# bfs18/nsynth_wavenet

Hardware: AMD Instinct MI355X
Metric: 16 kHz audio samples/sec, parallel-WaveNet (IAF student) generation (higher is better)
Workload: dtype split-fp16: activations stored as fp16 hi+lo pairs (32 bits per value, 22-bit significand, fp16 exponent range), contractions as 3 fp16 MFMAs per product with fp32 accumulate; conditioning term and outputs fp32; 1 GPU; BASELINE.json configs[1]: parallel_wavenet.json IAF student generation, synthetic 80-dim mel, 16 kHz, 1 utterance(s) of 384 frames = 76800 samples per GPU per step; batch_per_gpu=1, frames=384, samples_per_utterance=76800, weights=random-init (TF initialisers), seed 1234; noise drawn on device (Philox), precision=f16x3, parallelism=utterance-sharded x1 (no data-path collective)

## Files before the change

nsynth_wavenet_amd/csrc/wn_deconv.hip:

```cpp
#include <algorithm>

#include "wn_internal.h"
#include "wn_codec.h"
#include "wn_pack_h.h"
#include "wn_mfma_h.h"


namespace {

constexpr int DC_NT = 4;
constexpr int DC_QT = 16 * DC_NT;
constexpr int DC_XOFF = 8;
constexpr int DC_QW = 256;
constexpr int DH_KC = 4;

__host__ __device__ inline int dc_row_stride(int L) {
    return DC_XOFF + ((L + 5 + DC_QW - 1) / DC_QW) * DC_QW + 8;
}

__global__ void mel_to_cm_kernel(const float* __restrict__ mel, float* __restrict__ out,
                                 int F, int C, int xs) {
    const int b = blockIdx.z, c = blockIdx.y;
    const int col = blockIdx.x * blockDim.x + threadIdx.x;
    if (col >= xs) return;
    const int f = col - DC_XOFF;
    float v = 0.f;
    if (f >= 0 && f < F) v = mel[((size_t)b * F + f) * C + c];
    out[((size_t)b * C + c) * xs + col] = v;
}

__device__ inline float apply_act(float v, int act) {
    if (act == WN_ACT_LEAKY_RELU) return fmaxf(v, 0.4f * v);
    if (act == WN_ACT_RELU) return fmaxf(v, 0.f);
    return tanhf(v);
}

__global__ __launch_bounds__(256) void deconv_mfma_kernel(
    const float* __restrict__ x, int cin, int xs, const float* __restrict__ wp,
    float* __restrict__ yp, int cout, int Qp, int S, int taps, int zc_count) {
    const int lane = threadIdx.x & 63, wave = threadIdx.x >> 6;
    const int n = lane & 15, kq = lane >> 4;
    const int r = blockIdx.y;
    const int b = blockIdx.z / zc_count, zc = blockIdx.z % zc_count;
    const int cg = zc * 4 + wave;
    if (cg * 64 >= cout) return;
    const int q0 = blockIdx.x * DC_QT;
    const int nmb = cout / 16;
    const int cblk = cin / 16;
    const int nks4 = taps * cblk;

    f4 acc[4][DC_NT];
#pragma unroll
    for (int mb = 0; mb < 4; ++mb)
#pragma unroll
        for (int e = 0; e < DC_NT; ++e) acc[mb][e] = (f4){0.f, 0.f, 0.f, 0.f};

    const f4* wpr = reinterpret_cast<const f4*>(wp) + ((size_t)r * nks4 * nmb + cg * 4) * 64 + lane;
    const float* xb = x + (size_t)b * cin * xs + DC_XOFF + q0 + DC_NT * n;

    auto load = [&](int it, f4 (&a)[4], f4 (&bv)[4]) {
        const int j = it / cblk, c4 = it - j * cblk;
#pragma unroll
        for (int mb = 0; mb < 4; ++mb) a[mb] = wpr[((size_t)it * nmb + mb) * 64];
#pragma unroll
        for (int jj = 0; jj < 4; ++jj)
            bv[jj] = *reinterpret_cast<const f4u*>(xb + (size_t)(16 * c4 + 4 * jj + kq) * xs - j);
    };
    f4 a1[4], b1[4];
    load(0, a1, b1);
    for (int it = 0; it < nks4; ++it) {
        f4 a[4], bv[4];
#pragma unroll
        for (int i = 0; i < 4; ++i) { a[i] = a1[i]; bv[i] = b1[i]; }
        if (it + 1 < nks4) load(it + 1, a1, b1);
#pragma unroll
        for (int jj = 0; jj < 4; ++jj)
#pragma unroll
            for (int mb = 0; mb < 4; ++mb)
#pragma unroll
                for (int e = 0; e < DC_NT; ++e)
                    acc[mb][e] = __builtin_amdgcn_mfma_f32_16x16x4f32(a[mb][jj], bv[jj][e], acc[mb][e], 0, 0, 0);
    }
#pragma unroll
    for (int mb = 0; mb < 4; ++mb)
#pragma unroll
        for (int rr = 0; rr < 4; ++rr) {
            const int co = 64 * cg + 16 * mb + 4 * kq + rr;
            float* row = yp + (((size_t)b * S + r) * cout + co) * Qp + q0 + DC_NT * n;
            *reinterpret_cast<f4*>(row) = (f4){acc[mb][0][rr], acc[mb][1][rr], acc[mb][2][rr], acc[mb][3][rr]};
        }
}

constexpr int DI_MAXS = 32;
__global__ __launch_bounds__(256) void deconv_interleave_kernel(
    const float* __restrict__ yp, const float* __restrict__ bias, float* __restrict__ y,
    int cout, int Qp, int64_t ys, int yoff, int L, int S, int pL, int act) {
    __shared__ float tile[DI_MAXS][DC_QT + 1];
    const int co = blockIdx.y, b = blockIdx.z;
    const int q0 = blockIdx.x * DC_QT;
    for (int i = threadIdx.x; i < S * DC_QT; i += 256) {
        const int r = i / DC_QT, q = i - r * DC_QT;
        tile[r][q] = yp[(((size_t)b * S + r) * cout + co) * Qp + q0 + q];
    }
    __syncthreads();
    const float bco = bias[co];
    const int64_t SL = (int64_t)S * L;
    float* yr = y + ((size_t)b * cout + co) * ys + yoff;
    const int64_t n0 = (int64_t)S * q0 - pL;
    for (int i = threadIdx.x; i < S * DC_QT; i += 256) {
        const int q = i / S, r = i - q * S;
        const int64_t nn = n0 + i;
        if (nn >= 0 && nn < SL) yr[nn] = apply_act(tile[r][q] + bco, act);
    }
}

__global__ void mel_to_split_kernel(const float* __restrict__ mel, unsigned* __restrict__ out,
                                    int F, int C, int xs, unsigned* __restrict__ status) {
    const int b = blockIdx.z, cp = blockIdx.y;
    const int col = blockIdx.x * blockDim.x + threadIdx.x;
    if (col >= xs) return;
    const int f = col - DC_XOFF;
    unsigned hw = 0, lw = 0;
    if (f >= 0 && f < F) {
        const float* m = mel + ((size_t)b * F + f) * C + 2 * cp;
        float amax = 0.f;
        wn_split_pair_t(m[0], m[1], hw, lw, amax);
        wn_range_flag(amax, status);
    }
    out[((size_t)b * C + cp) * xs + col] = hw;
    out[((size_t)b * C + C / 2 + cp) * xs + col] = lw;
}

template <bool G4IN>
__global__ __launch_bounds__(256, 2) void deconv_mfma_h_kernel(
    const unsigned* __restrict__ x, int cin, int xs, const unsigned* __restrict__ wp,
    float* __restrict__ yp, int cout, int Qp, int S, int taps, float inv_scale) {
    __shared__ __attribute__((aligned(16))) unsigned lds[2][DH_KC * 4 * 512];
    const int lane = threadIdx.x & 63, wave = threadIdx.x >> 6;
    const int n = lane & 15, kg = lane >> 4;
    const int r = blockIdx.y;
    const int ncg = cout / 64;
    const int b = blockIdx.z / ncg, cg = blockIdx.z % ncg;
    const int q0 = blockIdx.x * DC_QW + wave * DC_QT;
    const int nmb = cout / 16;
    const int nb16 = cin / 16;
    const int nks = taps * nb16 / 2;
    const int nchunk = (nks + DH_KC - 1) / DH_KC;

    f4 acc[4][DC_NT];
#pragma unroll
    for (int mb = 0; mb < 4; ++mb)
#pragma unroll
        for (int e = 0; e < DC_NT; ++e) acc[mb][e] = (f4){0.f, 0.f, 0.f, 0.f};

    const wn_u4* wsrc = reinterpret_cast<const wn_u4*>(wp);
    auto stage = [&](int chunk, int buf) {
#pragma unroll
        for (int kl = 0; kl < DH_KC; ++kl) {
            const int ks = chunk * DH_KC + kl;
            if (ks < nks) {
                const wn_u4* src = wsrc + (((size_t)r * nks + ks) * nmb + cg * 4) * 128;
                wn_u4* dst = reinterpret_cast<wn_u4*>(lds[buf]) + kl * 512;
                dst[threadIdx.x] = src[threadIdx.x];
                dst[threadIdx.x + 256] = src[threadIdx.x + 256];
            }
        }
    };
    const unsigned* xb = x + (size_t)b * cin * xs;
    const size_t lo_plane = (size_t)(cin / 2) * xs;
    auto loadB = [&](int ks, wn_u4 (&vh)[DC_NT], wn_u4 (&vl)[DC_NT]) {
        if (G4IN) {
            const int nb32 = cin / 32;
            const int j = ks / nb32, c = ks - j * nb32;
            const unsigned* p = xb + ((size_t)(4 * c + kg) * xs + DC_XOFF + q0 + DC_NT * n - j) * 4;
#pragma unroll
            for (int e = 0; e < DC_NT; ++e) {
                vh[e] = *reinterpret_cast<const wn_u4*>(p + 4 * e);
                vl[e] = *reinterpret_cast<const wn_u4*>(p + lo_plane + 4 * e);
            }
        } else {
            wn_u4 bh[4], bl[4];
#pragma unroll
            for (int i = 0; i < 4; ++i) {
                const int g = 2 * ks + (i >> 1);
                const int j = g / nb16, blk = g - j * nb16;
                const unsigned* p = xb + (size_t)(8 * blk + 2 * kg + (i & 1)) * xs + DC_XOFF + q0 + DC_NT * n - j;
                bh[i] = *reinterpret_cast<const wn_u4 __attribute__((aligned(4)))*>(p);
                bl[i] = *reinterpret_cast<const wn_u4 __attribute__((aligned(4)))*>(p + lo_plane);
            }
#pragma unroll
            for (int e = 0; e < DC_NT; ++e) {
                vh[e] = (wn_u4){bh[0][e], bh[1][e], bh[2][e], bh[3][e]};
                vl[e] = (wn_u4){bl[0][e], bl[1][e], bl[2][e], bl[3][e]};
            }
        }
    };

    stage(0, 0);
    wn_u4 b1h[DC_NT], b1l[DC_NT];
    loadB(0, b1h, b1l);
    __syncthreads();
    for (int chunk = 0; chunk < nchunk; ++chunk) {
        const int buf = chunk & 1;
        if (chunk + 1 < nchunk) stage(chunk + 1, buf ^ 1);
        const wn_u4* Al = reinterpret_cast<const wn_u4*>(lds[buf]) + lane;
#pragma unroll
        for (int kl = 0; kl < DH_KC; ++kl) {
            const int ks = chunk * DH_KC + kl;
            if (ks >= nks) break;
            wn_u4 vh[DC_NT], vl[DC_NT];
#pragma unroll
            for (int e = 0; e < DC_NT; ++e) { vh[e] = b1h[e]; vl[e] = b1l[e]; }
            if (ks + 1 < nks) loadB(ks + 1, b1h, b1l);
#pragma unroll
            for (int mb = 0; mb < 4; ++mb) {
                const wn_u4 ah = Al[(kl * 4 + mb) * 128], al = Al[(kl * 4 + mb) * 128 + 64];
#pragma unroll
                for (int e = 0; e < DC_NT; ++e) {
                    f4 c = acc[mb][e];
                    c = __builtin_amdgcn_mfma_f32_16x16x32_f16(__builtin_bit_cast(wn_h8, ah), __builtin_bit_cast(wn_h8, vh[e]), c, 0, 0, 0);
                    c = __builtin_amdgcn_mfma_f32_16x16x32_f16(__builtin_bit_cast(wn_h8, ah), __builtin_bit_cast(wn_h8, vl[e]), c, 0, 0, 0);
                    c = __builtin_amdgcn_mfma_f32_16x16x32_f16(__builtin_bit_cast(wn_h8, al), __builtin_bit_cast(wn_h8, vh[e]), c, 0, 0, 0);
                    acc[mb][e] = c;
                }
            }
        }
        __syncthreads();
    }
#pragma unroll
    for (int mb = 0; mb < 4; ++mb)
#pragma unroll
        for (int rr = 0; rr < 4; ++rr) {
            const int co = 64 * cg + 16 * mb + 4 * kg + rr;
            float* row = yp + (((size_t)b * S + r) * cout + co) * Qp + q0 + DC_NT * n;
            *reinterpret_cast<f4*>(row) = (f4){acc[mb][0][rr] * inv_scale, acc[mb][1][rr] * inv_scale,
                                               acc[mb][2][rr] * inv_scale, acc[mb][3][rr] * inv_scale};
        }
}

__device__ inline unsigned dpp_shr1(unsigned old, unsigned src) {
    return (unsigned)__builtin_amdgcn_update_dpp((int)old, (int)src, 0x111, 0xf, 0xf, false);
}

template <int TAPS>
__global__ __launch_bounds__(256, 2) void deconv_mfma_hs_kernel(
    const unsigned* __restrict__ x, int cin, int xs, const unsigned* __restrict__ wp,
    float* __restrict__ yp, int cout, int Qp, int S, float inv_scale) {
    constexpr int taps = TAPS, NH = TAPS > 1 ? TAPS - 1 : 1;
    __shared__ __attribute__((aligned(16))) unsigned lds[2][DH_KC * 4 * 512];
    const int lane = threadIdx.x & 63, wave = threadIdx.x >> 6;
    const int n = lane & 15, kg = lane >> 4;
    const int r = blockIdx.y;
    const int ncg = cout / 64;
    const int b = blockIdx.z / ncg, cg = blockIdx.z % ncg;
    const int q0 = blockIdx.x * DC_QW + wave * DC_QT;
    const int nmb = cout / 16;
    const int nb32 = cin / 32;
    const int nks = taps * nb32;
    constexpr int ntg = (taps + DH_KC - 1) / DH_KC;
    const int nchunk = nb32 * ntg;

    f4 acc[4][DC_NT];
#pragma unroll
    for (int mb = 0; mb < 4; ++mb)
#pragma unroll
        for (int e = 0; e < DC_NT; ++e) acc[mb][e] = (f4){0.f, 0.f, 0.f, 0.f};

    const wn_u4* wsrc = reinterpret_cast<const wn_u4*>(wp);
    wn_u4 wt[DH_KC][2];
    auto stage_load = [&](int chunk) {
        const int c = chunk / ntg, tg = chunk - c * ntg;
#pragma unroll
        for (int kl = 0; kl < DH_KC; ++kl) {
            const int j = tg * DH_KC + kl;
            if (j < taps) {
                const wn_u4* src = wsrc + (((size_t)r * nks + j * nb32 + c) * nmb + cg * 4) * 128;
                wt[kl][0] = src[threadIdx.x];
                wt[kl][1] = src[threadIdx.x + 256];
            }
        }
    };
    auto stage_store = [&](int chunk, int buf) {
        const int c = chunk / ntg, tg = chunk - c * ntg;
#pragma unroll
        for (int kl = 0; kl < DH_KC; ++kl) {
            if (tg * DH_KC + kl < taps) {
                wn_u4* dst = reinterpret_cast<wn_u4*>(lds[buf]) + kl * 512;
                dst[threadIdx.x] = wt[kl][0];
                dst[threadIdx.x + 256] = wt[kl][1];
            }
        }
    };
    const unsigned* xb = x + (size_t)b * cin * xs;
    const size_t lo_plane = (size_t)(cin / 2) * xs;
    auto loadB = [&](int c, wn_u4 (&vh)[DC_NT], wn_u4 (&vl)[DC_NT], wn_u4 (&hh)[NH], wn_u4 (&hl)[NH]) {
        const unsigned* row = xb + ((size_t)(4 * c + kg) * xs + DC_XOFF + q0) * 4;
        const unsigned* p = row + DC_NT * n * 4;
#pragma unroll
        for (int e = 0; e < DC_NT; ++e) {
            vh[e] = *reinterpret_cast<const wn_u4*>(p + 4 * e);
            vl[e] = *reinterpret_cast<const wn_u4*>(p + lo_plane + 4 * e);
        }
#pragma unroll
        for (int k = 0; k + 1 < taps; ++k) {
            hh[k] = *reinterpret_cast<const wn_u4*>(row - 4 * (k + 1));
            hl[k] = *reinterpret_cast<const wn_u4*>(row + lo_plane - 4 * (k + 1));
        }
    };

    stage_load(0);
    stage_store(0, 0);
    wn_u4 nh[DC_NT], nl[DC_NT], nhh[NH], nhl[NH];
    loadB(0, nh, nl, nhh, nhl);
    __syncthreads();
    wn_u4 vh[DC_NT], vl[DC_NT], hh[NH], hl[NH];
    for (int c = 0; c < nb32; ++c) {
#pragma unroll
        for (int e = 0; e < DC_NT; ++e) { vh[e] = nh[e]; vl[e] = nl[e]; }
#pragma unroll
        for (int k = 0; k < NH; ++k) { hh[k] = nhh[k]; hl[k] = nhl[k]; }
        if (c + 1 < nb32) loadB(c + 1, nh, nl, nhh, nhl);
#pragma unroll
      for (int tg = 0; tg < ntg; ++tg) {
        const int chunk = c * ntg + tg;
        const int buf = chunk & 1;
        if (chunk + 1 < nchunk) stage_load(chunk + 1);
        const wn_u4* Al = reinterpret_cast<const wn_u4*>(lds[buf]) + lane;
#pragma unroll
        for (int kl = 0; kl < DH_KC; ++kl) {
            const int j = tg * DH_KC + kl;
            if (j < taps) {
            if (j > 0) {
                const wn_u4 th = vh[DC_NT - 1], tl = vl[DC_NT - 1];
#pragma unroll
                for (int e = DC_NT - 1; e > 0; --e) { vh[e] = vh[e - 1]; vl[e] = vl[e - 1]; }
                const wn_u4 oh = hh[j > 0 ? j - 1 : 0], ol = hl[j > 0 ? j - 1 : 0];
#pragma unroll
                for (int i = 0; i < 4; ++i) {
                    vh[0][i] = dpp_shr1(oh[i], th[i]);
                    vl[0][i] = dpp_shr1(ol[i], tl[i]);
                }
            }
#pragma unroll
            for (int mb = 0; mb < 4; ++mb) {
                const wn_u4 ah = Al[(kl * 4 + mb) * 128], al = Al[(kl * 4 + mb) * 128 + 64];
#pragma unroll
                for (int e = 0; e < DC_NT; ++e) {
                    f4 cc = acc[mb][e];
                    cc = __builtin_amdgcn_mfma_f32_16x16x32_f16(__builtin_bit_cast(wn_h8, ah), __builtin_bit_cast(wn_h8, vh[e]), cc, 0, 0, 0);
                    cc = __builtin_amdgcn_mfma_f32_16x16x32_f16(__builtin_bit_cast(wn_h8, ah), __builtin_bit_cast(wn_h8, vl[e]), cc, 0, 0, 0);
                    cc = __builtin_amdgcn_mfma_f32_16x16x32_f16(__builtin_bit_cast(wn_h8, al), __builtin_bit_cast(wn_h8, vh[e]), cc, 0, 0, 0);
                    acc[mb][e] = cc;
                }
            }
            }
        }
        if (chunk + 1 < nchunk) stage_store(chunk + 1, buf ^ 1);
        __syncthreads();
      }
    }
#pragma unroll
    for (int mb = 0; mb < 4; ++mb)
#pragma unroll
        for (int rr = 0; rr < 4; ++rr) {
            const int co = 64 * cg + 16 * mb + 4 * kg + rr;
            float* row = yp + (((size_t)b * S + r) * cout + co) * Qp + q0 + DC_NT * n;
            *reinterpret_cast<f4*>(row) = (f4){acc[mb][0][rr] * inv_scale, acc[mb][1][rr] * inv_scale,
                                               acc[mb][2][rr] * inv_scale, acc[mb][3][rr] * inv_scale};
        }
}

constexpr int PG_TP = 4;
constexpr int PG_NT = 5;
constexpr int PG_WAVES = 8;
constexpr int PG_FRAMES = PG_WAVES * 16 * PG_NT;
constexpr int PG_KS_WORDS = 8 * 2 * 64 * 4;
constexpr int PG_RG_WORDS_PER_BLOCK = PG_TP * PG_KS_WORDS;
constexpr int PG_LDS_BYTES = 2 * PG_RG_WORDS_PER_BLOCK * 4;
constexpr int PG_MAXG = 8;

struct PgArgs {
    const unsigned* x;
    int cin, xs, L;
    const unsigned* wp;
    const float* bias;
    float inv_scale;
    unsigned* y;
    int cout, S, act;
    int64_t ys;
    int yoff;
    unsigned* status;
    int ntiles;
    int ngroups, nrg;
    int g_p0[PG_MAXG], g_nph[PG_MAXG], g_d[PG_MAXG], g_rg0[PG_MAXG];
};

__device__ inline void pg_dma16(const unsigned* gsrc, unsigned lds_byte_addr) {
    unsigned keep;
    asm volatile("s_mov_b32 %0, m0\n\ts_mov_b32 m0, %2\n\ts_nop 0\n\tglobal_load_lds_dwordx4 %1, off\n\ts_mov_b32 m0, %0"
                 : "=&s"(keep) : "v"(gsrc), "s"(__builtin_amdgcn_readfirstlane(lds_byte_addr)) : "memory");
}

__global__ __launch_bounds__(PG_WAVES * 64, 1) void deconv_pg_kernel(const PgArgs A) {
    extern __shared__ __attribute__((aligned(16))) unsigned pg_lds[];
    char* lds = reinterpret_cast<char*>(pg_lds);
    const unsigned lds_base = __builtin_amdgcn_readfirstlane((unsigned)(size_t)(__attribute__((address_space(3))) char*)lds);
    constexpr int NT = PG_NT, TP = PG_TP, NR = NT + TP - 1;
    int rg, tile;
    if ((A.nrg & 7) == 0) {
        const int k = blockIdx.x >> 3;
        rg = (blockIdx.x & 7) + 8 * (k / A.ntiles);
        tile = k % A.ntiles;
    } else {
        rg = blockIdx.x / A.ntiles;
        tile = blockIdx.x % A.ntiles;
    }
    int gi = 0;
    for (int k = 1; k < A.ngroups; ++k) if (rg >= A.g_rg0[k]) gi = k;
    const int p0 = A.g_p0[gi], nph = A.g_nph[gi], dcol = A.g_d[gi], sub = rg - A.g_rg0[gi];
    const int b = blockIdx.y;
    const int lane = threadIdx.x & 63, wave = __builtin_amdgcn_readfirstlane(threadIdx.x >> 6);
    const int n = lane & 15, kg = lane >> 4;
    const int nb32 = A.cin / 32, ngi = A.cin / 8, ngo = A.cout / 8;
    const int f0 = tile * PG_FRAMES + wave * (16 * NT);
    const unsigned* wsrc = A.wp + (size_t)rg * nb32 * PG_RG_WORDS_PER_BLOCK;

    f4 acc[8][NT];
#pragma unroll
    for (int mb = 0; mb < 8; ++mb)
#pragma unroll
        for (int e = 0; e < NT; ++e) acc[mb][e] = (f4){0.f, 0.f, 0.f, 0.f};

    auto stage = [&](int c, int buf) {
        const unsigned* src = wsrc + (size_t)c * PG_RG_WORDS_PER_BLOCK;
#pragma unroll
        for (int i = 0; i < PG_RG_WORDS_PER_BLOCK / 256 / PG_WAVES; ++i) {
            const int piece = wave * (PG_RG_WORDS_PER_BLOCK / 256 / PG_WAVES) + i;
            pg_dma16(src + (size_t)(piece * 64 + lane) * 4, lds_base + buf * (PG_RG_WORDS_PER_BLOCK * 4) + piece * 1024);
        }
    };
    const __amdgpu_buffer_rsrc_t rx = __builtin_amdgcn_make_buffer_rsrc(
        (void*)(A.x + (size_t)b * 2 * ngi * A.xs * 4), 0, 2 * ngi * A.xs * 16, 0x00020000);
    const int lo_plane = ngi * A.xs * 16;
    wn_u4 Rh[NR], Rl[NR];
    auto loadB = [&](int c) {
        const int vo = (4 * c + kg) * A.xs * 16 + (DC_XOFF + f0 + NT * n + dcol - (TP - 1)) * 16;
#pragma unroll
        for (int k = 0; k < NR; ++k) {
            Rh[k] = __builtin_bit_cast(wn_u4, __builtin_amdgcn_raw_buffer_load_b128(rx, vo + k * 16, 0, 0));
            Rl[k] = __builtin_bit_cast(wn_u4, __builtin_amdgcn_raw_buffer_load_b128(rx, vo + k * 16, lo_plane, 0));
        }
    };

    stage(0, 0);
    loadB(0);
    asm volatile("s_waitcnt vmcnt(0)" ::: "memory");
    __syncthreads();
    for (int c = 0; c < nb32; ++c) {
        const int buf = c & 1;
        if (c + 1 < nb32) stage(c + 1, buf ^ 1);
#pragma unroll
        for (int m = 0; m < TP; ++m) {
            const wn_u4* Al = reinterpret_cast<const wn_u4*>(lds + buf * (PG_RG_WORDS_PER_BLOCK * 4)) + m * (PG_KS_WORDS / 4) + lane;
#pragma unroll
            for (int mb = 0; mb < 8; ++mb) {
                const wn_u4 ah = Al[mb * 128], al = Al[mb * 128 + 64];
#pragma unroll
                for (int e = 0; e < NT; ++e) {
                    const wn_u4 bh = Rh[e + TP - 1 - m], bl = Rl[e + TP - 1 - m];
                    f4 cc = acc[mb][e];
                    cc = __builtin_amdgcn_mfma_f32_16x16x32_f16(__builtin_bit_cast(wn_h8, ah), __builtin_bit_cast(wn_h8, bh), cc, 0, 0, 0);
                    cc = __builtin_amdgcn_mfma_f32_16x16x32_f16(__builtin_bit_cast(wn_h8, ah), __builtin_bit_cast(wn_h8, bl), cc, 0, 0, 0);
                    cc = __builtin_amdgcn_mfma_f32_16x16x32_f16(__builtin_bit_cast(wn_h8, al), __builtin_bit_cast(wn_h8, bh), cc, 0, 0, 0);
                    acc[mb][e] = cc;
                }
            }
        }
        if (c + 1 < nb32) loadB(c + 1);
        asm volatile("s_waitcnt vmcnt(0)" ::: "memory");
        __syncthreads();
    }
    const __amdgpu_buffer_rsrc_t ry = __builtin_amdgcn_make_buffer_rsrc(
        (void*)(A.y + (size_t)b * 2 * ngo * A.ys * 4), 0, (int)(2 * ngo * A.ys * 16), 0x00020000);
    const int lo_out = (int)(ngo * A.ys * 16);
    float amax = 0.f;
    const bool half = nph == 2;
    const int cb_first = half ? 4 * sub : 2 * sub;
    float bs[4][4];
#pragma unroll
    for (int k = 0; k < 4; ++k)
#pragma unroll
        for (int rr = 0; rr < 4; ++rr) bs[k][rr] = (half || k < 2) ? A.bias[16 * (cb_first + k) + 4 * kg + rr] : 0.f;
    char* patch = lds + wave * 8192;
    const int fr = f0 + NT * (lane >> 2);
    const int w2r = lane & 3;
    const int phr = half ? (w2r & 1) : w2r, sgr = half ? (w2r >> 1) : 0;
#pragma unroll
    for (int e = 0; e < NT; ++e) {
#pragma unroll
        for (int w2 = 0; w2 < 4; ++w2) {
            wn_u4 hw, lw;
#pragma unroll
            for (int slot = 0; slot < 4; ++slot) {
                const int blk = slot >> 1, r0 = (slot & 1) * 2;
                const float a0 = half ? acc[(4 * (w2 & 1) + 2 * (w2 >> 1) + blk) & 7][e][r0] : acc[(2 * w2 + blk) & 7][e][r0];
                const float a1 = half ? acc[(4 * (w2 & 1) + 2 * (w2 >> 1) + blk) & 7][e][r0 + 1] : acc[(2 * w2 + blk) & 7][e][r0 + 1];
                const float b0 = half ? bs[2 * (w2 >> 1) + blk][r0] : bs[blk][r0];
                const float b1 = half ? bs[2 * (w2 >> 1) + blk][r0 + 1] : bs[blk][r0 + 1];
                const float v0 = apply_act(fmaf(a0, A.inv_scale, b0), A.act);
                const float v1 = apply_act(fmaf(a1, A.inv_scale, b1), A.act);
                unsigned a, c2;
                wn_split_pair_t(v0, v1, a, c2, amax);
                hw[slot] = a;
                lw[slot] = c2;
            }
            *reinterpret_cast<wn_u4*>(patch + ((kg * 16 + n) * 4 + w2) * 16) = hw;
            *reinterpret_cast<wn_u4*>(patch + 4096 + ((kg * 16 + n) * 4 + w2) * 16) = lw;
        }
        const int f = fr + e;
        const int64_t tcol = A.yoff + (int64_t)A.S * f + p0 + phr;
#pragma unroll
        for (int kr = 0; kr < 4; ++kr) {
            const int g = 4 * ((cb_first >> 1) + sgr) + kr;
            const int vo = f < A.L ? (int)(((int64_t)g * A.ys + tcol) * 16) : (int)0x80000000;
            const wn_u4 hw = *reinterpret_cast<const wn_u4*>(patch + (kr * 64 + lane) * 16);
            const wn_u4 lw = *reinterpret_cast<const wn_u4*>(patch + 4096 + (kr * 64 + lane) * 16);
            buf_st4(hw, ry, vo, 0);
            buf_st4(lw, ry, vo, lo_out);
        }
    }
    wn_range_flag(amax, A.status);
}

__global__ void cm_to_tm_kernel(const float* __restrict__ in, float* __restrict__ out,
                                int C, int64_t T, int64_t cs) {
    __shared__ float tile[32][33];
    const int b = blockIdx.z;
    const int64_t t0 = (int64_t)blockIdx.x * 32;
    const int c0 = blockIdx.y * 32;
    const int tx = threadIdx.x & 31, ty = threadIdx.x >> 5;
    for (int i = ty; i < 32; i += 8) {
        const int c = c0 + i;
        const int64_t t = t0 + tx;
        tile[i][tx] = (c < C && t < T) ? in[((size_t)b * C + c) * cs + t] : 0.f;
    }
    __syncthreads();
    for (int i = ty; i < 32; i += 8) {
        const int64_t t = t0 + i;
        const int c = c0 + tx;
        if (t < T && c < C) out[((size_t)b * T + t) * C + c] = tile[tx][i];
    }
}

constexpr int DG_Q = 32;
template <int SC>
__global__ __launch_bounds__(256) void deconv_interleave_g4_kernel(
    const float* __restrict__ yp, const float* __restrict__ bias, unsigned* __restrict__ y,
    int cout, int Qp, int64_t ys, int yoff, int L, int S_rt, int pL, int act, unsigned* __restrict__ status,
    int zero_pads) {
    const int S = SC ? SC : S_rt;
    __shared__ float tile[8][DI_MAXS][DG_Q + 1];
    const int g = blockIdx.y, b = blockIdx.z;
    const int q0 = blockIdx.x * DG_Q;
    if (zero_pads && (blockIdx.x == 0 || blockIdx.x + 1 == gridDim.x)) {
        wn_u4* rh = reinterpret_cast<wn_u4*>(y + ((size_t)b * cout * ys)) + (size_t)g * ys;
        wn_u4* rl = rh + (size_t)(cout / 8) * ys;
        const int64_t lo = blockIdx.x == 0 ? 0 : yoff + (int64_t)S * L, hi = blockIdx.x == 0 ? yoff : ys;
        for (int64_t i = lo + threadIdx.x; i < hi; i += 256) rh[i] = rl[i] = (wn_u4){0u, 0u, 0u, 0u};
    }
    const int prbase = 16 * (g >> 2) + 2 * (g & 3);
    for (int i = threadIdx.x; i < 8 * S * (DG_Q / 4); i += 256) {
        const int c8 = i / (S * (DG_Q / 4)), j = i - c8 * S * (DG_Q / 4);
        const int r = j / (DG_Q / 4), q = 4 * (j - r * (DG_Q / 4));
        const int slot = c8 >> 1;
        const int ch = 2 * (prbase + 8 * (slot >> 1) + (slot & 1)) + (c8 & 1);
        const f4 v = *reinterpret_cast<const f4*>(yp + (((size_t)b * S + r) * cout + ch) * Qp + q0 + q);
#pragma unroll
        for (int k = 0; k < 4; ++k) tile[c8][r][q + k] = v[k];
    }
    __syncthreads();
    float bs[8];
#pragma unroll
    for (int c8 = 0; c8 < 8; ++c8) {
        const int slot = c8 >> 1;
        bs[c8] = bias[2 * (prbase + 8 * (slot >> 1) + (slot & 1)) + (c8 & 1)];
    }
    const int ng = cout / 8;
    const int64_t SL = (int64_t)S * L;
    wn_u4* yh = reinterpret_cast<wn_u4*>(y + ((size_t)b * cout * ys)) + (size_t)g * ys + yoff;
    wn_u4* yl = yh + (size_t)ng * ys;
    const int64_t n0 = (int64_t)S * q0 - pL;
    float amax = 0.f;
    for (int i = threadIdx.x; i < S * DG_Q; i += 256) {
        const int q = i / S, r = i - q * S;
        const int64_t nn = n0 + i;
        if (nn >= 0 && nn < SL) {
            wn_u4 hw, lw;
#pragma unroll
            for (int slot = 0; slot < 4; ++slot) {
                unsigned a, c2;
                wn_split_pair_t(apply_act(tile[2 * slot][r][q] + bs[2 * slot], act),
                                apply_act(tile[2 * slot + 1][r][q] + bs[2 * slot + 1], act), a, c2, amax);
                hw[slot] = a;
                lw[slot] = c2;
            }
            yh[nn] = hw;
            yl[nn] = lw;
        }
    }
    wn_range_flag(amax, status);
}

constexpr int DF_WAVES = 8;
constexpr int DF_CIN = 80;
constexpr int DF_NKS = 4 * (DF_CIN / 16) / 2;
constexpr int DF_WIN = 16 + 3;
constexpr int DF_PF = 3;

__device__ inline float mul_round_add(float a, float s, float b) {
#pragma clang fp contract(off)
    const float m = a * s;
    return m + b;
}

struct FrontArgs {
    const float* mel;
    int B, F;
    const unsigned* wp;
    const float* bias;
    float inv_scale;
    unsigned* y;
    int ys;
    int S, pL, act;
    int ncb, nunits;
    unsigned* status;
};

__global__ __launch_bounds__(DF_WAVES * 64) void deconv_front_kernel(const FrontArgs A) {
    __shared__ __attribute__((aligned(16))) unsigned win[2][DF_WIN][DF_CIN / 2];
    const int u = (blockIdx.x & 7) * (gridDim.x >> 3) + (blockIdx.x >> 3);
    if (u >= A.nunits) return;
    const int cb = u % A.ncb, pb = u / A.ncb;
    const int b = pb % A.B, p = pb / A.B;
    const int r = (p + A.pL) % A.S, d = (p + A.pL) / A.S;
    const int lane = threadIdx.x & 63, wave = __builtin_amdgcn_readfirstlane(threadIdx.x >> 6);
    const int n = lane & 15, kg = lane >> 4;
    const int f0 = 16 * cb;
    constexpr int ng = 32, nmb = 16;

    const float* melb = A.mel + (size_t)b * A.F * DF_CIN;
    constexpr int NP = (DF_WIN * (DF_CIN / 2) + DF_WAVES * 64 - 1) / (DF_WAVES * 64);
    wn_f2 mv[NP];
    bool mok[NP];
#pragma unroll
    for (int k = 0; k < NP; ++k) {
        const int i = threadIdx.x + k * DF_WAVES * 64;
        const int fl = i / (DF_CIN / 2), pr = i - fl * (DF_CIN / 2);
        const int fr = f0 + d - 3 + fl;
        mok[k] = fl < DF_WIN && fr >= 0 && fr < A.F;
        mv[k] = *reinterpret_cast<const wn_f2 __attribute__((aligned(4)))*>(melb + (size_t)min(max(fr, 0), A.F - 1) * DF_CIN + 2 * pr);
    }
    f4 bs[2];
#pragma unroll
    for (int mb = 0; mb < 2; ++mb) bs[mb] = *reinterpret_cast<const f4u*>(A.bias + 32 * wave + 16 * mb + 4 * kg);
    const wn_u4* wsrc = reinterpret_cast<const wn_u4*>(A.wp) + ((size_t)r * DF_NKS * nmb + 2 * wave) * 128 + lane;
    wn_u4 ah[DF_NKS][2], al[DF_NKS][2];
    auto loadA = [&](int ks) {
#pragma unroll
        for (int mb = 0; mb < 2; ++mb) {
            ah[ks][mb] = wsrc[(ks * nmb + mb) * 128];
            al[ks][mb] = wsrc[(ks * nmb + mb) * 128 + 64];
        }
        __builtin_amdgcn_sched_barrier(0);
    };
#pragma unroll
    for (int ks = 0; ks < DF_PF; ++ks) loadA(ks);
    float amax = 0.f;
#pragma unroll
    for (int k = 0; k < NP; ++k) {
        const int i = threadIdx.x + k * DF_WAVES * 64;
        const int fl = i / (DF_CIN / 2), pr = i - fl * (DF_CIN / 2);
        if (fl < DF_WIN) {
            unsigned hw = 0, lw = 0;
            if (mok[k]) wn_split_pair_t(mv[k].x, mv[k].y, hw, lw, amax);
            win[0][fl][pr] = hw;
            win[1][fl][pr] = lw;
        }
    }
    __syncthreads();

    f4 acc[2];
    acc[0] = acc[1] = (f4){0.f, 0.f, 0.f, 0.f};
#pragma unroll
    for (int ks = 0; ks < DF_NKS; ++ks) {
        if (ks + DF_PF < DF_NKS) loadA(ks + DF_PF);
        wn_u4 vh, vl;
#pragma unroll
        for (int i = 0; i < 4; ++i) {
            const int g = 2 * ks + (i >> 1);
            const int j = g / (DF_CIN / 16), blk = g - j * (DF_CIN / 16);
            vh[i] = win[0][n + 3 - j][8 * blk + 2 * kg + (i & 1)];
            vl[i] = win[1][n + 3 - j][8 * blk + 2 * kg + (i & 1)];
        }
#pragma unroll
        for (int mb = 0; mb < 2; ++mb) {
            f4 c = acc[mb];
            c = __builtin_amdgcn_mfma_f32_16x16x32_f16(__builtin_bit_cast(wn_h8, ah[ks][mb]), __builtin_bit_cast(wn_h8, vh), c, 0, 0, 0);
            c = __builtin_amdgcn_mfma_f32_16x16x32_f16(__builtin_bit_cast(wn_h8, ah[ks][mb]), __builtin_bit_cast(wn_h8, vl), c, 0, 0, 0);
            c = __builtin_amdgcn_mfma_f32_16x16x32_f16(__builtin_bit_cast(wn_h8, al[ks][mb]), __builtin_bit_cast(wn_h8, vh), c, 0, 0, 0);
            acc[mb] = c;
        }
    }

    const __amdgpu_buffer_rsrc_t ry = __builtin_amdgcn_make_buffer_rsrc(
        (void*)(A.y + (size_t)b * 2 * ng * A.ys * 4), 0, 2 * ng * A.ys * 16, 0x00020000);
    const int lo_out = ng * A.ys * 16;
    wn_u4 hw, lw;
#pragma unroll
    for (int slot = 0; slot < 4; ++slot) {
        const int mb = slot >> 1, r0 = (slot & 1) * 2;
        const float v0 = apply_act(mul_round_add(acc[mb][r0], A.inv_scale, bs[mb][r0]), A.act);
        const float v1 = apply_act(mul_round_add(acc[mb][r0 + 1], A.inv_scale, bs[mb][r0 + 1]), A.act);
        unsigned a, c2;
        wn_split_pair_t(v0, v1, a, c2, amax);
        hw[slot] = a;
        lw[slot] = c2;
    }
    const int f = f0 + n;
    {
        const int vo = f < A.F ? ((4 * wave + kg) * A.ys + DC_XOFF + A.S * f + p) * 16 : (int)0x80000000;
        buf_st4(hw, ry, vo, 0);
        buf_st4(lw, ry, vo, lo_out);
    }
    wn_range_flag(amax, A.status);
    if (cb + 1 == A.ncb) {
        const int SL = A.S * A.F, nz = A.ys - SL;
        for (int row = p; row < 2 * ng; row += A.S)
            for (int i = threadIdx.x; i < nz; i += DF_WAVES * 64)
                buf_st4((wn_u4){0u, 0u, 0u, 0u}, ry, (row * A.ys + (i < DC_XOFF ? i : SL + i)) * 16, 0);
    }
}

}

int wn_pack_deconv(wn_handle* h, std::vector<float>& blob) {
    const wn_config& c = h->cfg;
    for (auto& sp : h->stacks) {
        int cin = c.n_mel;
        for (int j = 0; j < c.n_deconv; ++j) {
            DeconvLayerPack lp;
            lp.cin = cin;
            lp.cout = c.deconv_width;
            lp.K = c.deconv_filter[j];
            lp.S = c.deconv_stride[j];
            lp.pL = (lp.K - lp.S) / 2;
            lp.taps = lp.K / lp.S;
            if (cin % 16) return wn_fail(h, WN_EINVAL, "deconv: input channels %d not a multiple of 16", cin);
            std::string scope = (sp.prefix.empty() ? std::string() : sp.prefix + "/") +
                                (c.use_resize_conv ? "resize_conv_" : "trans_conv_") + std::to_string(j + 1);
            std::vector<float> W;
            if (c.use_resize_conv) {
                const int fl = lp.K, S = lp.S;
                std::vector<float> Wr = wn_get_kernel(h, scope, "W", false);
                int taps = (fl - 1 + S - 1) / S + 1;
                if ((taps * (cin / 16)) % 2) ++taps;
                lp.taps = taps;
                lp.K = S * taps;
                lp.pL = fl - 1 - (fl - 1) / 2;
                W.assign((size_t)lp.K * lp.cout * cin, 0.f);
                for (int r = 0; r < S; ++r)
                    for (int k = 0; k < fl; ++k) {
                        const int m = r + k - (fl - 1);
                        const int jt = m >= 0 ? 0 : (-m + S - 1) / S;
                        for (int co = 0; co < lp.cout; ++co)
                            for (int ci = 0; ci < cin; ++ci)
                                W[((size_t)(S * jt + r) * lp.cout + co) * cin + ci] +=
                                    Wr[((size_t)k * cin + ci) * lp.cout + co];
                    }
            } else {
                W = wn_get_kernel(h, scope, "kernel", true);
            }
            const std::vector<float>& bias = h->vars.at(scope + (c.use_resize_conv ? "/biases" : "/bias")).data;
            const int nmb = lp.cout / 16, cblk = cin / 16, nks4 = lp.taps * cblk;
            blob.resize(align_up(blob.size(), 64));
// ... 388 lines not shown
```

Measured before the change: 64.91 million samples/s.

## Interleave next-chunk register loads with MFMA taps in deconv main loop

After: 64.97 million samples/s, median of 6. Within noise of the previous version (+0.1%).

```diff
diff --git a/nsynth_wavenet_amd/csrc/wn_deconv.hip b/nsynth_wavenet_amd/csrc/wn_deconv.hip
--- a/nsynth_wavenet_amd/csrc/wn_deconv.hip
+++ b/nsynth_wavenet_amd/csrc/wn_deconv.hip
@@ -395,10 +395,10 @@
     int g_p0[PG_MAXG], g_nph[PG_MAXG], g_d[PG_MAXG], g_rg0[PG_MAXG];
 };
 
-__device__ inline void pg_dma16(const unsigned* gsrc, unsigned lds_byte_addr) {
+__device__ inline void pg_dma16(const unsigned* sbase, unsigned lane_byte_off, unsigned lds_byte_addr) {
     unsigned keep;
-    asm volatile("s_mov_b32 %0, m0\n\ts_mov_b32 m0, %2\n\ts_nop 0\n\tglobal_load_lds_dwordx4 %1, off\n\ts_mov_b32 m0, %0"
-                 : "=&s"(keep) : "v"(gsrc), "s"(__builtin_amdgcn_readfirstlane(lds_byte_addr)) : "memory");
+    asm volatile("s_mov_b32 %0, m0\n\ts_mov_b32 m0, %3\n\ts_nop 0\n\tglobal_load_lds_dwordx4 %1, %2\n\ts_mov_b32 m0, %0"
+                 : "=&s"(keep) : "v"(lane_byte_off), "s"(sbase), "s"(__builtin_amdgcn_readfirstlane(lds_byte_addr)) : "memory");
 }
 
 __global__ __launch_bounds__(PG_WAVES * 64, 1) void deconv_pg_kernel(const PgArgs A) {
@@ -436,49 +436,64 @@
 #pragma unroll
         for (int i = 0; i < PG_RG_WORDS_PER_BLOCK / 256 / PG_WAVES; ++i) {
             const int piece = wave * (PG_RG_WORDS_PER_BLOCK / 256 / PG_WAVES) + i;
-            pg_dma16(src + (size_t)(piece * 64 + lane) * 4, lds_base + buf * (PG_RG_WORDS_PER_BLOCK * 4) + piece * 1024);
+            pg_dma16(src + (size_t)piece * 256, lane * 16, lds_base + buf * (PG_RG_WORDS_PER_BLOCK * 4) + piece * 1024);
         }
     };
     const __amdgpu_buffer_rsrc_t rx = __builtin_amdgcn_make_buffer_rsrc(
         (void*)(A.x + (size_t)b * 2 * ngi * A.xs * 4), 0, 2 * ngi * A.xs * 16, 0x00020000);
     const int lo_plane = ngi * A.xs * 16;
     wn_u4 Rh[NR], Rl[NR];
-    auto loadB = [&](int c) {
-        const int vo = (4 * c + kg) * A.xs * 16 + (DC_XOFF + f0 + NT * n + dcol - (TP - 1)) * 16;
-#pragma unroll
-        for (int k = 0; k < NR; ++k) {
-            Rh[k] = __builtin_bit_cast(wn_u4, __builtin_amdgcn_raw_buffer_load_b128(rx, vo + k * 16, 0, 0));
-            Rl[k] = __builtin_bit_cast(wn_u4, __builtin_amdgcn_raw_buffer_load_b128(rx, vo + k * 16, lo_plane, 0));
-        }
+    constexpr int OOB = 0x40000000;
+    const int vo0 = kg * A.xs * 16 + (DC_XOFF + f0 + NT * n + dcol - (TP - 1)) * 16;
+    auto loadR = [&](int c, int k) {
+        const int vo = vo0 + 4 * c * A.xs * 16 + k * 16 + (c < nb32 ? 0 : OOB);
+        Rh[k] = __builtin_bit_cast(wn_u4, __builtin_amdgcn_raw_buffer_load_b128(rx, vo, 0, 0));
+        Rl[k] = __builtin_bit_cast(wn_u4, __builtin_amdgcn_raw_buffer_load_b128(rx, vo, lo_plane, 0));
+        __builtin_amdgcn_sched_barrier(0);
     };
+    auto mfma_tap = [&](int m, int mb, int e, const wn_u4& ah, const wn_u4& al) {
+        const wn_u4 bh = Rh[e + TP - 1 - m], bl = Rl[e + TP - 1 - m];
+        f4 cc = acc[mb][e];
+        cc = __builtin_amdgcn_mfma_f32_16x16x32_f16(__builtin_bit_cast(wn_h8, ah), __builtin_bit_cast(wn_h8, bh), cc, 0, 0, 0);
+        cc = __builtin_amdgcn_mfma_f32_16x16x32_f16(__builtin_bit_cast(wn_h8, ah), __builtin_bit_cast(wn_h8, bl), cc, 0, 0, 0);
+        cc = __builtin_amdgcn_mfma_f32_16x16x32_f16(__builtin_bit_cast(wn_h8, al), __builtin_bit_cast(wn_h8, bh), cc, 0, 0, 0);
+        acc[mb][e] = cc;
+    };
 
     stage(0, 0);
-    loadB(0);
+#pragma unroll
+    for (int k = 0; k < NR; ++k) loadR(0, k);
     asm volatile("s_waitcnt vmcnt(0)" ::: "memory");
     __syncthreads();
+    auto tap_part = [&](const wn_u4* Al, int m, int e0, int e1, int rot) {
+#pragma unroll
+        for (int mb = 0; mb < 8; ++mb) {
+            const wn_u4 ah = Al[mb * 128], al = Al[mb * 128 + 64];
+#pragma unroll
+            for (int i = 0; i < e1 - e0; ++i) mfma_tap(m, mb, e0 + (i + rot) % (e1 - e0), ah, al);
+        }
+    };
+    constexpr int EH3 = 3;
     for (int c = 0; c < nb32; ++c) {
         const int buf = c & 1;
+        const wn_u4* Ab = reinterpret_cast<const wn_u4*>(lds + buf * (PG_RG_WORDS_PER_BLOCK * 4)) + lane;
+        tap_part(Ab, 0, 0, NT, 2);
+        loadR(c + 1, NR - 1);
         if (c + 1 < nb32) stage(c + 1, buf ^ 1);
-#pragma unroll
-        for (int m = 0; m < TP; ++m) {
-            const wn_u4* Al = reinterpret_cast<const wn_u4*>(lds + buf * (PG_RG_WORDS_PER_BLOCK * 4)) + m * (PG_KS_WORDS / 4) + lane;
-#pragma unroll
-            for (int mb = 0; mb < 8; ++mb) {
-                const wn_u4 ah = Al[mb * 128], al = Al[mb * 128 + 64];
-#pragma unroll
-                for (int e = 0; e < NT; ++e) {
-                    const wn_u4 bh = Rh[e + TP - 1 - m], bl = Rl[e + TP - 1 - m];
-                    f4 cc = acc[mb][e];
-                    cc = __builtin_amdgcn_mfma_f32_16x16x32_f16(__builtin_bit_cast(wn_h8, ah), __builtin_bit_cast(wn_h8, bh), cc, 0, 0, 0);
-                    cc = __builtin_amdgcn_mfma_f32_16x16x32_f16(__builtin_bit_cast(wn_h8, ah), __builtin_bit_cast(wn_h8, bl), cc, 0, 0, 0);
-                    cc = __builtin_amdgcn_mfma_f32_16x16x32_f16(__builtin_bit_cast(wn_h8, al), __builtin_bit_cast(wn_h8, bh), cc, 0, 0, 0);
-                    acc[mb][e] = cc;
-                }
-            }
-        }
-        if (c + 1 < nb32) loadB(c + 1);
-        asm volatile("s_waitcnt vmcnt(0)" ::: "memory");
-        __syncthreads();
+        tap_part(Ab + PG_KS_WORDS / 4, 1, 0, NT, 0);
+        loadR(c + 1, NR - 2);
+        tap_part(Ab + 2 * (PG_KS_WORDS / 4), 2, 0, NT, 0);
+        loadR(c + 1, NR - 3);
+        tap_part(Ab + 3 * (PG_KS_WORDS / 4), 3, 0, EH3, 0);
+        asm volatile("" ::: "memory");
+#pragma unroll
+        for (int k = 0; k < EH3; ++k) loadR(c + 1, k);
+        tap_part(Ab + 3 * (PG_KS_WORDS / 4), 3, EH3, NT, 0);
+#pragma unroll
+        for (int k = EH3; k < NT; ++k) loadR(c + 1, k);
+        asm volatile("s_waitcnt vmcnt(4)" ::: "memory");
+        __builtin_amdgcn_s_barrier();
+        asm volatile("" ::: "memory");
     }
     const __amdgpu_buffer_rsrc_t ry = __builtin_amdgcn_make_buffer_rsrc(
         (void*)(A.y + (size_t)b * 2 * ngo * A.ys * 4), 0, (int)(2 * ngo * A.ys * 16), 0x00020000);
```

## Software-pipeline deconv main loop with per-slot window reloads and scheduled MFMA groups

Applied to the files above, without the earlier changes.

Result: no change. 66.09 million samples/s before, 66.12 million samples/s after (median of 6 runs) (+0.0%).

```diff
diff --git a/nsynth_wavenet_amd/csrc/wn_deconv.hip b/nsynth_wavenet_amd/csrc/wn_deconv.hip
--- a/nsynth_wavenet_amd/csrc/wn_deconv.hip
+++ b/nsynth_wavenet_amd/csrc/wn_deconv.hip
@@ -1,4 +1,6 @@
 #include <algorithm>
+#include <type_traits>
+#include <utility>
 
 #include "wn_internal.h"
 #include "wn_codec.h"
@@ -378,6 +380,46 @@
 constexpr int PG_RG_WORDS_PER_BLOCK = PG_TP * PG_KS_WORDS;
 constexpr int PG_LDS_BYTES = 2 * PG_RG_WORDS_PER_BLOCK * 4;
 constexpr int PG_MAXG = 8;
+constexpr int PG_DMA_PER_WAVE = PG_RG_WORDS_PER_BLOCK / 256 / PG_WAVES;
+constexpr int PG_STEPS = 40;
+constexpr int PG_DMA_STEP = 3;
+constexpr int pg_step_tap(int s) { return s < 24 ? s / 8 : PG_TP - 1; }
+constexpr int pg_step_e0(int s) { return s >= 24 && s < 32 ? 3 : 0; }
+constexpr int pg_step_e1(int s) { return s >= 32 ? 3 : PG_NT; }
+constexpr int pg_slot_reload_step(int k) { return k == 7 ? 7 : k == 6 ? 15 : k == 5 ? 23 : k >= 3 ? 31 : PG_STEPS - 1; }
+constexpr bool pg_step_reads_slot(int s, int k) {
+    return k >= pg_step_e0(s) + PG_TP - 1 - pg_step_tap(s) && k < pg_step_e1(s) + PG_TP - 1 - pg_step_tap(s);
+}
+constexpr bool pg_reloads_are_dead() {
+    for (int k = 0; k < PG_NT + PG_TP - 1; ++k)
+        for (int s = pg_slot_reload_step(k) + 1; s < PG_STEPS; ++s)
+            if (pg_step_reads_slot(s, k)) return false;
+    return true;
+}
+constexpr bool pg_steps_cover_the_tile() {
+    for (int m = 0; m < PG_TP; ++m)
+        for (int e = 0; e < PG_NT; ++e) {
+            int n = 0;
+            for (int s = 0; s < PG_STEPS; s += 8) n += pg_step_tap(s) == m && e >= pg_step_e0(s) && e < pg_step_e1(s);
+            if (n != 1) return false;
+        }
+    return true;
+}
+static_assert(PG_TP == 4 && PG_NT == 5, "the step table above is written for four taps and five column blocks");
+static_assert(pg_reloads_are_dead(),"a window slot is reloaded in front of a step of the same stage that reads it");
+static_assert(pg_steps_cover_the_tile(), "the steps do not cover (tap, column block) exactly once");
+static_assert(PG_STEPS % 2 == 0, "the fragment pairs rotate with the step parity across stages");
+constexpr int pg_slots_reloaded_behind(int s) {
+    int n = 0;
+    for (int k = 0; k < PG_NT + PG_TP - 1; ++k) n += pg_slot_reload_step(k) == s;
+    return n;
+}
+template <int... S, class F>
+__device__ inline void pg_static_for(std::integer_sequence<int, S...>, F&& f) {
+    (f(std::integral_constant<int, S>{}), ...);
+}
+constexpr int PG_B_LOADS = 2 * (PG_NT + PG_TP - 1);
+static_assert(PG_DMA_STEP < pg_slot_reload_step(PG_NT + PG_TP - 2), "a window reload is issued in front of the LDS-DMA requests");
 
 struct PgArgs {
     const unsigned* x;
@@ -432,54 +474,82 @@
         for (int e = 0; e < NT; ++e) acc[mb][e] = (f4){0.f, 0.f, 0.f, 0.f};
 
     auto stage = [&](int c, int buf) {
-        const unsigned* src = wsrc + (size_t)c * PG_RG_WORDS_PER_BLOCK;
-#pragma unroll
-        for (int i = 0; i < PG_RG_WORDS_PER_BLOCK / 256 / PG_WAVES; ++i) {
-            const int piece = wave * (PG_RG_WORDS_PER_BLOCK / 256 / PG_WAVES) + i;
-            pg_dma16(src + (size_t)(piece * 64 + lane) * 4, lds_base + buf * (PG_RG_WORDS_PER_BLOCK * 4) + piece * 1024);
-        }
+        const unsigned* src = wsrc + (size_t)c * PG_RG_WORDS_PER_BLOCK + wave * (PG_DMA_PER_WAVE * 256);
+#pragma unroll
+        for (int i = 0; i < PG_DMA_PER_WAVE; ++i)
+            pg_dma16(src + i * 256 + lane * 4, lds_base + buf * (PG_RG_WORDS_PER_BLOCK * 4) + (wave * PG_DMA_PER_WAVE + i) * 1024);
     };
     const __amdgpu_buffer_rsrc_t rx = __builtin_amdgcn_make_buffer_rsrc(
         (void*)(A.x + (size_t)b * 2 * ngi * A.xs * 4), 0, 2 * ngi * A.xs * 16, 0x00020000);
     const int lo_plane = ngi * A.xs * 16;
     wn_u4 Rh[NR], Rl[NR];
-    auto loadB = [&](int c) {
-        const int vo = (4 * c + kg) * A.xs * 16 + (DC_XOFF + f0 + NT * n + dcol - (TP - 1)) * 16;
-#pragma unroll
-        for (int k = 0; k < NR; ++k) {
-            Rh[k] = __builtin_bit_cast(wn_u4, __builtin_amdgcn_raw_buffer_load_b128(rx, vo + k * 16, 0, 0));
-            Rl[k] = __builtin_bit_cast(wn_u4, __builtin_amdgcn_raw_buffer_load_b128(rx, vo + k * 16, lo_plane, 0));
-        }
+    const int vo0 = kg * A.xs * 16 + (DC_XOFF + f0 + NT * n + dcol - (TP - 1)) * 16, vo_step = 4 * A.xs * 16;
+    int vo = vo0;
+    auto loadB = [&](int k) {
+        Rh[k] = __builtin_bit_cast(wn_u4, __builtin_amdgcn_raw_buffer_load_b128(rx, vo + k * 16, 0, 0));
+        Rl[k] = __builtin_bit_cast(wn_u4, __builtin_amdgcn_raw_buffer_load_b128(rx, vo + k * 16, lo_plane, 0));
     };
+    const wn_u4* Al = reinterpret_cast<const wn_u4*>(lds) + lane;
+    wn_u4 ah[2], al[2];
+    auto loadA = [&](int buf, int s) {
+        const wn_u4* p = Al + buf * (PG_RG_WORDS_PER_BLOCK / 4) + pg_step_tap(s) * (PG_KS_WORDS / 4) + (s & 7) * 128;
+        ah[s & 1] = p[0];
+        al[s & 1] = p[64];
+    };
 
     stage(0, 0);
-    loadB(0);
+#pragma unroll
+    for (int k = NR - 1; k >= 0; --k)
+        if (pg_slot_reload_step(k) != PG_STEPS - 1) loadB(k);
+    __builtin_amdgcn_sched_barrier(0);
+#pragma unroll
+    for (int k = NR - 1; k >= 0; --k)
+        if (pg_slot_reload_step(k) == PG_STEPS - 1) loadB(k);
     asm volatile("s_waitcnt vmcnt(0)" ::: "memory");
     __syncthreads();
-    for (int c = 0; c < nb32; ++c) {
+    auto run_stage = [&](int c, auto last) {
+        constexpr bool LAST = decltype(last)::value;
         const int buf = c & 1;
-        if (c + 1 < nb32) stage(c + 1, buf ^ 1);
-#pragma unroll
-        for (int m = 0; m < TP; ++m) {
-            const wn_u4* Al = reinterpret_cast<const wn_u4*>(lds + buf * (PG_RG_WORDS_PER_BLOCK * 4)) + m * (PG_KS_WORDS / 4) + lane;
-#pragma unroll
-            for (int mb = 0; mb < 8; ++mb) {
-                const wn_u4 ah = Al[mb * 128], al = Al[mb * 128 + 64];
-#pragma unroll
-                for (int e = 0; e < NT; ++e) {
-                    const wn_u4 bh = Rh[e + TP - 1 - m], bl = Rl[e + TP - 1 - m];
-                    f4 cc = acc[mb][e];
-                    cc = __builtin_amdgcn_mfma_f32_16x16x32_f16(__builtin_bit_cast(wn_h8, ah), __builtin_bit_cast(wn_h8, bh), cc, 0, 0, 0);
-                    cc = __builtin_amdgcn_mfma_f32_16x16x32_f16(__builtin_bit_cast(wn_h8, ah), __builtin_bit_cast(wn_h8, bl), cc, 0, 0, 0);
-                    cc = __builtin_amdgcn_mfma_f32_16x16x32_f16(__builtin_bit_cast(wn_h8, al), __builtin_bit_cast(wn_h8, bh), cc, 0, 0, 0);
-                    acc[mb][e] = cc;
-                }
-            }
-        }
-        if (c + 1 < nb32) loadB(c + 1);
-        asm volatile("s_waitcnt vmcnt(0)" ::: "memory");
+        if constexpr (!LAST) vo += vo_step;
+        loadA(buf, 0);
+        pg_static_for(std::make_integer_sequence<int, PG_STEPS>{}, [&](auto step) {
+            constexpr int s = decltype(step)::value;
+            constexpr int m = pg_step_tap(s), mb = s & 7, e0 = pg_step_e0(s), e1 = pg_step_e1(s);
+            if constexpr (s + 1 < PG_STEPS) loadA(buf, s + 1);
+            constexpr int nld = s == 0 || LAST ? 0 : 2 * pg_slots_reloaded_behind(s - 1);
+#pragma unroll
+            for (int k = NR - 1; k >= 0; --k)
+                if (!LAST && s > 0 && pg_slot_reload_step(k) == s - 1) loadB(k);
+            const wn_h8 fh = __builtin_bit_cast(wn_h8, ah[s & 1]), fl = __builtin_bit_cast(wn_h8, al[s & 1]);
+#pragma unroll
+            for (int e = e0; e < e1; ++e)
+                acc[mb][e] = __builtin_amdgcn_mfma_f32_16x16x32_f16(fh, __builtin_bit_cast(wn_h8, Rh[e + TP - 1 - m]), acc[mb][e], 0, 0, 0);
+#pragma unroll
+            for (int e = e0; e < e1; ++e)
+                acc[mb][e] = __builtin_amdgcn_mfma_f32_16x16x32_f16(fh, __builtin_bit_cast(wn_h8, Rl[e + TP - 1 - m]), acc[mb][e], 0, 0, 0);
+#pragma unroll
+            for (int e = e0; e < e1; ++e)
+                acc[mb][e] = __builtin_amdgcn_mfma_f32_16x16x32_f16(fl, __builtin_bit_cast(wn_h8, Rh[e + TP - 1 - m]), acc[mb][e], 0, 0, 0);
+            if constexpr (s + 1 < PG_STEPS) __builtin_amdgcn_sched_group_barrier(0x100, s == 0 ? 4 : 2, 0);
+            if constexpr (nld > 0) __builtin_amdgcn_sched_group_barrier(0x020, nld, 0);
+            __builtin_amdgcn_sched_group_barrier(0x008, 3 * (e1 - e0), 0);
+            if constexpr (s == PG_DMA_STEP) {
+                __builtin_amdgcn_sched_barrier(0);
+                asm volatile("s_waitcnt vmcnt(0)" ::"v"(Rh[2]), "v"(Rl[2]) : "memory");
+                if constexpr (!LAST) stage(c + 1, buf ^ 1);
+                __builtin_amdgcn_sched_barrier(0);
+            }
+        });
+        if constexpr (!LAST) {
+#pragma unroll
+            for (int k = NR - 1; k >= 0; --k)
+                if (pg_slot_reload_step(k) == PG_STEPS - 1) loadB(k);
+            asm volatile("s_waitcnt vmcnt(%0)" ::"n"(PG_B_LOADS) : "memory");
+        }
         __syncthreads();
-    }
+    };
+    for (int c = 0; c + 1 < nb32; ++c) run_stage(c, std::false_type{});
+    run_stage(nb32 - 1, std::true_type{});
     const __amdgpu_buffer_rsrc_t ry = __builtin_amdgcn_make_buffer_rsrc(
         (void*)(A.y + (size_t)b * 2 * ngo * A.ys * 4), 0, (int)(2 * ngo * A.ys * 16), 0x00020000);
     const int lo_out = (int)(ngo * A.ys * 16);
```
